# junejunejune/c_orb_slam

Measured on AMD Instinct MI355X. Metric: tracking FPS + ORB matches/sec, KITTI-00 stereo; local-BA iter/sec, higher is better.
Workload: dtype u8

## Files before the change

c_orb_slam_amd/csrc/orb_extract.hip:

```cpp
#include "orb_extract.hpp"

#include <algorithm>
#include <atomic>
#include <chrono>
#include <cmath>
#include <cstring>
#include <thread>

namespace orbgpu {

__constant__ int8_t c_pattern[256 * 4];
__constant__ int8_t c_disc[2 * 1024];
__constant__ int c_ndisc;
__constant__ int c_umax[16];
__constant__ int c_gauss[7];

static const int8_t kPattern[256 * 4] = {
#include "brief_pattern.inc"
};

__device__ __forceinline__ int xcd_tile(int bid, int nb) { return (bid & 7) * (nb >> 3) + (bid >> 3); }
static inline unsigned grid8(int n) { return (unsigned)((n + 7) & ~7); }
constexpr int kFastSplitLevel = 3;

// ... 286 lines not shown
        __syncthreads();
        const int nch = L.pitch >> 4;
        for (int t = tid; t < st.w * nch; t += 256) {
            const int ri = t / nch, ch = t - ri * nch;
            const int py = rl[ri];
            const int y = refl101(py - kEdge, L.h);
            const uint8_t* row = cur + min(max(y - st.x, 0), nrows - 1) * L.rp;
            const int x0 = ch * 16 - kEdge;
            uint4 o;
            if (x0 >= 1 && x0 + 16 <= L.w) {
                const uint32_t* w = reinterpret_cast<const uint32_t*>(row + x0 - 1);
                const uint32_t w0 = w[0], w1 = w[1], w2 = w[2], w3 = w[3], w4 = w[4];
                o.x = __builtin_amdgcn_alignbyte(w1, w0, 1);
                o.y = __builtin_amdgcn_alignbyte(w2, w1, 1);
                o.z = __builtin_amdgcn_alignbyte(w3, w2, 1);
                o.w = __builtin_amdgcn_alignbyte(w4, w3, 1);
            } else {
                uint32_t q[4] = {0, 0, 0, 0};
#pragma unroll
                for (int j = 0; j < 16; j++) q[j >> 2] |= (uint32_t)row[refl101(x0 + j, L.w)] << (8 * (j & 3));
                o = make_uint4(q[0], q[1], q[2], q[3]);
            }
            *reinterpret_cast<uint4*>(base + L.off + (size_t)py * L.pitch + 16 * ch) = o;
        }
        rl += st.w;
        prev = cur;
        prev_lo = st.x;
        prev_rp = L.rp;
        prev_n = nrows;
    }
    (void)src_w;
}

constexpr int BT_W = 128, BT_H = 32, BT_LW = BT_W + 8;
typedef unsigned short ushort2v __attribute__((ext_vector_type(2)));
__device__ __forceinline__ uint32_t dot2u(uint32_t pair, uint32_t taps, uint32_t acc) {
    return __builtin_amdgcn_udot2(__builtin_bit_cast(ushort2v, pair), __builtin_bit_cast(ushort2v, taps), acc, false);
}
__global__ void __launch_bounds__(256) k_blur7(const uint8_t* __restrict__ pyr, uint8_t* __restrict__ blur,
                                               size_t img_bytes, size_t blur_bytes,
                                               const BlurTile* __restrict__ tiles, int ntiles) {
    constexpr int WPR = BT_LW / 4;
    constexpr int SR = BT_H + 6;
    __shared__ uint32_t s_src[SR * WPR];
    __shared__ uint4 s_pair[(SR / 2) * (BT_W / 4)];
    const int tile = xcd_tile(blockIdx.x, gridDim.x);
    if (tile >= ntiles) return;
    const BlurTile tl = tiles[tile];
    const int b = blockIdx.y;
    const uint8_t* P = pyr + (size_t)b * img_bytes + tl.off;
    uint8_t* O = blur + (size_t)b * blur_bytes + tl.boff;
    const int x0 = tl.tx * BT_W, y0 = tl.ty * BT_H;
    {
        constexpr int NU = (SR * WPR + 255) / 256;
        uint32_t v[NU];
#pragma unroll
        for (int u = 0; u < NU; u++) {
            const int i = threadIdx.x + 256 * u;
            const int r = i / WPR, wq = i - r * WPR;
            const int yy = min(y0 + r - 3, tl.h + 2) + kEdge;
            const int c = min(kEdge - 3 + x0 + 4 * wq, tl.pitch - 4);
            v[u] = i < SR * WPR ? *reinterpret_cast<const uint32_t*>(P + (size_t)yy * tl.pitch + c) : 0u;
        }
#pragma unroll
        for (int u = 0; u < NU; u++)
            if (threadIdx.x + 256 * u < SR * WPR) s_src[threadIdx.x + 256 * u] = v[u];
    }
    const uint32_t TLO = (uint32_t)c_gauss[0] | ((uint32_t)c_gauss[1] << 8) | ((uint32_t)c_gauss[2] << 16) |
                         ((uint32_t)c_gauss[3] << 24);
    const uint32_t THI = (uint32_t)c_gauss[4] | ((uint32_t)c_gauss[5] << 8) | ((uint32_t)c_gauss[6] << 16);
    __syncthreads();
    for (int i = threadIdx.x; i < (SR / 2) * (BT_W / 4); i += 256) {
        const int pr = i / (BT_W / 4), q = i - pr * (BT_W / 4);
        uint32_t o[4];
#pragma unroll
        for (int h = 0; h < 2; h++) {
            const uint32_t* w = s_src + (2 * pr + h) * WPR + q;
            const uint32_t w0 = w[0], w1 = w[1], w2 = w[2];
#pragma unroll
            for (int j = 0; j < 4; j++) {
                const uint32_t lo = j ? __builtin_amdgcn_alignbyte(w1, w0, j) : w0;
                const uint32_t hi = j ? __builtin_amdgcn_alignbyte(w2, w1, j) : w1;
                const uint32_t r = __builtin_amdgcn_udot4(lo, TLO, __builtin_amdgcn_udot4(hi, THI, 0u, false), false);
                o[j] = h ? (o[j] | (r << 16)) : r;
            }
        }
        s_pair[i] = make_uint4(o[0], o[1], o[2], o[3]);
    }
    const uint32_t C01 = (uint32_t)c_gauss[0] | ((uint32_t)c_gauss[1] << 16);
    const uint32_t C23 = (uint32_t)c_gauss[2] | ((uint32_t)c_gauss[3] << 16);
    const uint32_t C45 = (uint32_t)c_gauss[4] | ((uint32_t)c_gauss[5] << 16);
    const uint32_t C6_ = (uint32_t)c_gauss[6];
    const uint32_t C_0 = (uint32_t)c_gauss[0] << 16;
    const uint32_t C12 = (uint32_t)c_gauss[1] | ((uint32_t)c_gauss[2] << 16);
    const uint32_t C34 = (uint32_t)c_gauss[3] | ((uint32_t)c_gauss[4] << 16);
    const uint32_t C56 = (uint32_t)c_gauss[5] | ((uint32_t)c_gauss[6] << 16);
    __syncthreads();
    for (int i = threadIdx.x; i < (BT_H / 2) * (BT_W / 4); i += 256) {
        const int p = i / (BT_W / 4), q = i - p * (BT_W / 4);
        const int y = y0 + 2 * p, x = x0 + 4 * q;
        if (y >= tl.h || x >= tl.w) continue;
        const uint4 a = s_pair[(p + 0) * (BT_W / 4) + q], bq = s_pair[(p + 1) * (BT_W / 4) + q];
        const uint4 c = s_pair[(p + 2) * (BT_W / 4) + q], d = s_pair[(p + 3) * (BT_W / 4) + q];
        const uint32_t A[4] = {a.x, a.y, a.z, a.w}, B[4] = {bq.x, bq.y, bq.z, bq.w};
        const uint32_t Cc[4] = {c.x, c.y, c.z, c.w}, D[4] = {d.x, d.y, d.z, d.w};
        uint32_t ev = 0, od = 0;
#pragma unroll
        for (int j = 0; j < 4; j++) {
            const uint32_t se = dot2u(D[j], C6_, dot2u(Cc[j], C45, dot2u(B[j], C23, dot2u(A[j], C01, 0u))));
            const uint32_t so = dot2u(D[j], C56, dot2u(Cc[j], C34, dot2u(B[j], C12, dot2u(A[j], C_0, 0u))));
            ev |= min((se + (1u << 15)) >> 16, 255u) << (8 * j);
            od |= min((so + (1u << 15)) >> 16, 255u) << (8 * j);
        }
        *reinterpret_cast<uint32_t*>(O + (size_t)y * tl.bpitch + x) = ev;
        if (y + 1 < tl.h) *reinterpret_cast<uint32_t*>(O + (size_t)(y + 1) * tl.bpitch + x) = od;
    }
}

constexpr int FC_LD = 76;
constexpr int FC_MAXR = 70;

typedef short short2v __attribute__((ext_vector_type(2)));
__device__ __forceinline__ short2v pk16(int lo, int hi) {
    short2v r;
    r.x = (short)lo;
    r.y = (short)hi;
    return r;
}
__device__ __forceinline__ uint32_t pk_bits(short2v v) { return __builtin_bit_cast(uint32_t, v); }
__device__ __forceinline__ short2v pk_min(short2v a, short2v b) { return __builtin_elementwise_min(a, b); }
__device__ __forceinline__ short2v pk_max(short2v a, short2v b) { return __builtin_elementwise_max(a, b); }

__device__ __forceinline__ short2v fast_score2_lds(const uint8_t* pa, const uint8_t* pb) {
    constexpr int ld = FC_LD;
    constexpr int ring[16] = {3 * ld,      3 * ld + 1,  2 * ld + 2,  ld + 3,  3,  -ld + 3, -2 * ld + 2, -3 * ld + 1,
                              -3 * ld,     -3 * ld - 1, -2 * ld - 2, -ld - 3, -3, ld - 3,  2 * ld - 2,  3 * ld - 1};
    const short2v v = pk16(pa[0], pb[0]);
    short2v d[16], mn2[16], mx2[16];
#pragma unroll
    for (int k = 0; k < 16; k++) d[k] = v - pk16(pa[ring[k]], pb[ring[k]]);
#pragma unroll
    for (int k = 0; k < 16; k++) {
        mn2[k] = pk_min(d[k], d[(k + 1) & 15]);
        mx2[k] = pk_max(d[k], d[(k + 1) & 15]);
    }
    short2v mn4[8], mx4[8];
#pragma unroll
    for (int k = 0; k < 8; k++) {
// ... 395 lines not shown
        scale_[i] = (float)(scale_[i - 1] * scaleFactorD_);
        sigma2_[i] = scale_[i] * scale_[i];
    }
    for (int i = 0; i < nlevels; i++) {
        invScale_[i] = 1.0f / scale_[i];
        invSigma2_[i] = 1.0f / sigma2_[i];
    }
    const float factor = (float)(1.0f / scaleFactorD_);
    float nDesired = nfeatures * (1 - factor) / (1 - (float)std::pow((double)factor, (double)nlevels));
    int sum = 0;
    for (int l = 0; l < nlevels - 1; l++) {
        nPerLevel_[l] = (int)cvRoundf_host(nDesired);
        sum += nPerLevel_[l];
        nDesired *= factor;
    }
    nPerLevel_[nlevels - 1] = std::max(nfeatures - sum, 0);
    umax_.assign(kHalfPatch + 1, 0);
    const int vmax = (int)std::floor(kHalfPatch * std::sqrt(2.f) / 2 + 1);
    const int vmin = (int)std::ceil(kHalfPatch * std::sqrt(2.f) / 2);
    const double hp2 = kHalfPatch * kHalfPatch;
    for (int v = 0; v <= vmax; ++v) umax_[v] = (int)std::lrint(std::sqrt(hp2 - v * v));
    for (int v = kHalfPatch, v0 = 0; v >= vmin; --v) {
        while (umax_[v0] == umax_[v0 + 1]) ++v0;
        umax_[v] = v0;
        ++v0;
    }
}

Extractor::~Extractor() { release(); }

void Extractor::release() {
    release_remap();
    auto F = [](void* p) { if (p) (void)hipFree(p); };
    F(d_in_); F(d_pyr_); F(d_blur_); F(d_slots_); F(d_counts_); F(d_cells_); F(d_tiles_); F(d_work_); F(d_groups_);
    F(d_lcb_); F(d_packed_); F(d_hdr_); F(d_sel_); F(d_levels_); F(d_tabs_);
    F(d_kps_); F(d_desc_); F(d_jobsel_); F(d_jobcnt_); F(d_octlv_); F(d_gscr_); F(d_nout_); F(d_ptiles_);
    F(d_chain_); F(d_cellslot_); F(d_flowcnt_);
    d_flowcnt_ = nullptr;
    d_ptiles_ = nullptr;
    d_chain_ = nullptr;
    d_cellslot_ = nullptr;
    d_jobsel_ = d_jobcnt_ = d_octlv_ = d_gscr_ = d_nout_ = nullptr;
    d_in_ = d_pyr_ = d_blur_ = nullptr;
    d_slots_ = nullptr; d_counts_ = nullptr; d_cells_ = nullptr; d_tiles_ = nullptr; d_work_ = nullptr; d_groups_ = nullptr;
    work_B_ = -1;
    d_lcb_ = nullptr; d_packed_ = nullptr; d_hdr_ = nullptr; d_gtotal_ = nullptr; d_sel_ = nullptr;
    d_levels_ = nullptr; d_tabs_ = nullptr; d_kps_ = nullptr; d_desc_ = nullptr;
    if (h_nout_) (void)hipHostFree(h_nout_);
    h_nout_ = nullptr;
    if (h_in_) (void)hipHostFree(h_in_);
    h_in_ = nullptr;
    h_in_cap_ = 0;
    for (auto& e : ev_) if (e) (void)hipEventDestroy(e);
    for (auto& e : ev_) e = nullptr;
    if (stream_ && ownStream_) (void)hipStreamDestroy(stream_);
    stream_ = nullptr;
    if (evBlur_) (void)hipEventDestroy(evBlur_);
    evBlur_ = nullptr;
    if (evPyrA_) (void)hipEventDestroy(evPyrA_);
    if (evFastA_) (void)hipEventDestroy(evFastA_);
    evPyrA_ = evFastA_ = nullptr;
    if (side_) (void)hipStreamDestroy(side_);
    side_ = nullptr;
}

int Extractor::init_device(int maxW, int maxH, int maxBatch) {
    int ndev = 0;
    if (hipGetDeviceCount(&ndev) != hipSuccess || ndev <= 0) return -4;
    if (const char* pe = getenv("ORBGPU_EXTRACT_STREAM_PRIO"); pe && pe[0] == '1') {
        int lo = 0, hi = 0;
        ORB_HIP_CHECK(hipDeviceGetStreamPriorityRange(&lo, &hi));
        ORB_HIP_CHECK(hipStreamCreateWithPriority(&stream_, hipStreamNonBlocking, hi));
    } else {
        ORB_HIP_CHECK(hipStreamCreateWithFlags(&stream_, hipStreamNonBlocking));
    }
    for (auto& e : ev_) ORB_HIP_CHECK(hipEventCreate(&e));
    const char* eb = getenv("ORBGPU_BLUR_SIDE");
    const char* ef = getenv("ORBGPU_FAST_SPLIT");
    const bool blurSide = eb && atoi(eb) > 0;
    fastSplit_ = ef && atoi(ef) == 1 && !blurSide;
    const char* ew = getenv("ORBGPU_PYR_FLOW");
    flow_ = ew && ew[0] == '1';
    if (blurSide || fastSplit_) ORB_HIP_CHECK(hipStreamCreateWithFlags(&side_, hipStreamNonBlocking));
    if (blurSide) ORB_HIP_CHECK(hipEventCreateWithFlags(&evBlur_, hipEventDisableTiming));
    if (fastSplit_) {
        ORB_HIP_CHECK(hipEventCreateWithFlags(&evPyrA_, hipEventDisableTiming));
        ORB_HIP_CHECK(hipEventCreateWithFlags(&evFastA_, hipEventDisableTiming));
    }
    static bool consts_done = false;
    if (!consts_done) {
        ORB_HIP_CHECK(hipMemcpyToSymbol(HIP_SYMBOL(c_pattern), kPattern, sizeof(kPattern)));
        int taps[7];
        gaussian_taps(taps);
        ORB_HIP_CHECK(hipMemcpyToSymbol(HIP_SYMBOL(c_gauss), taps, sizeof(taps)));
        consts_done = true;
    }
    std::vector<int8_t> disc;
    for (int v = -kHalfPatch; v <= kHalfPatch; v++) {
        const int d = v == 0 ? kHalfPatch : umax_[std::abs(v)];
        for (int u = -d; u <= d; u++) { disc.push_back((int8_t)u); disc.push_back((int8_t)v); }
    }
    const int nd = (int)disc.size() / 2;
    ORB_HIP_CHECK(hipMemcpyToSymbol(HIP_SYMBOL(c_disc), disc.data(), disc.size()));
    ORB_HIP_CHECK(hipMemcpyToSymbol(HIP_SYMBOL(c_ndisc), &nd, sizeof(int)));
    int um[16];
    for (int v = 0; v <= kHalfPatch; v++) um[v] = v == 0 ? kHalfPatch : umax_[v];
    ORB_HIP_CHECK(hipMemcpyToSymbol(HIP_SYMBOL(c_umax), um, sizeof(um)));
    maxW_ = maxW; maxH_ = maxH; maxB_ = maxBatch;
    return 0;
}

int Extractor::build_work(int B) {
    constexpr int kXcds = 8;
    const int ngroups = (int)groups_.size();
    std::vector<int> unit;
    for (int c = 0; c < ngroups; c++)
        if (c == 0 || groups_[c].lvl_off != groups_[c - 1].lvl_off || groups_[c].r0 != groups_[c - 1].r0)
            unit.push_back(c);
    unit.push_back(ngroups);
    const long long splitOff =
        nlevels_ > kFastSplitLevel ? (long long)levels_[kFastSplitLevel].off : std::numeric_limits<long long>::max();
    std::vector<int> work;
    for (int part = 0; part < 2; part++) {
        std::vector<std::vector<int>> lists(kXcds);
        long u = 0;
        for (int b = 0; b < B; b++)
            for (size_t k = 0; k + 1 < unit.size(); k++) {
                if ((groups_[unit[k]].lvl_off < splitOff) != (part == 0)) continue;
                for (int c = unit[k]; c < unit[k + 1]; c++) lists[u % kXcds].push_back((b << 16) | c);
                u++;
            }
        size_t len = 0;
        for (auto& l : lists) len = std::max(len, l.size());
        const size_t base = work.size();
        work.resize(base + len * kXcds, -1);
        for (int x = 0; x < kXcds; x++)
            for (size_t sl = 0; sl < lists[x].size(); sl++) work[base + sl * kXcds + x] = lists[x][sl];
        work_part_[part] = (int)(len * kXcds);
    }
    if (d_work_) (void)hipFree(d_work_);
    d_work_ = nullptr;
    ORB_HIP_CHECK(hipMalloc(&d_work_, std::max<size_t>(work.size(), 1) * 4));
// ... 312 lines not shown
        for (int j = 0; j < ncol;) {
            const CellDesc &a = cells_[cb + j];
            const bool two = j + 1 < ncol && spans(a.c0, a.c1, cells_[cb + j + 1].c0, cells_[cb + j + 1].c1);
            csel.push_back({j, two ? 2 : 1});
            j += two ? 2 : 1;
        }
        for (auto& rp : rsel)
            for (auto& cp : csel) {
                CellGroup g{};
                const CellDesc& tl = cells_[rowb[rp.first] + cp.first];
                const CellDesc& br = cells_[rowb[rp.first + rp.second - 1] + cp.first + cp.second - 1];
                g.r0 = tl.r0; g.c0 = tl.c0;
                g.rows = br.r1 - tl.r0; g.cols = br.c1 - tl.c0;
                g.rsplit = rp.second == 2 ? tl.r1 - tl.r0 - 6 : std::max(g.rows - 6, 0);
                g.csplit = cp.second == 2 ? tl.c1 - tl.c0 - 6 : std::max(g.cols - 6, 0);
                g.pitch = tl.pitch;
                g.lvl_off = tl.lvl_off;
                for (int k = 0; k < 4; k++) {
                    const int di = k >> 1, dj = k & 1;
                    g.cell[k] = -1;
                    if (di >= rp.second || dj >= cp.second) continue;
                    const int c = rowb[rp.first + di] + cp.first + dj;
                    const CellDesc& cd = cells_[c];
                    g.cell[k] = c;
                    g.cap[k] = cd.cap;
                    g.slot_off[k] = cd.slot_off;
                    g.xadd[k] = cd.offx - (cd.c0 - g.c0);
                    g.yadd[k] = cd.offy - (cd.r0 - g.r0);
                }
                groups_.push_back(g);
            }
    }
    if (groups_.size() > 65535) return -1;
    tiles_.clear();
    for (int l = 0; l < nlevels_; l++) {
        const LevelHost& L = levels_[l];
        for (int ty = 0; ty < (L.h + BT_H - 1) / BT_H; ty++)
            for (int tx = 0; tx < (L.w + BT_W - 1) / BT_W; tx++) {
                BlurTile t;
                t.off = L.off; t.pitch = L.pitch; t.w = L.w; t.h = L.h; t.tx = tx; t.ty = ty;
                t.boff = L.boff; t.bpitch = L.bpitch;
                tiles_.push_back(t);
            }
    }
    std::vector<uint8_t> tabs;
    auto push = [&tabs](const void* p, size_t n) -> size_t {
        size_t o = (tabs.size() + 15) & ~(size_t)15;
        tabs.resize(o + n);
        memcpy(tabs.data() + o, p, n);
        return o;
    };
    tab_off_.assign(nlevels_, {0, 0, 0, 0});
    std::vector<std::vector<int>> yrAll(nlevels_);
    xofsAll_.assign(nlevels_, {});
    xalAll_.assign(nlevels_, {});
    ptiles_.clear();
    ptile_begin_.assign(2 * (nlevels_ + 1), 0);
    ptile_n_.assign(2 * nlevels_, 0);
    plds_.assign(2 * nlevels_, 0);
    ptile_th_.assign(2 * nlevels_, 0);
    for (int l = 1; l < nlevels_; l++) {
        const int sw = levels_[l - 1].w, sh = levels_[l - 1].h, dw = levels_[l].w, dh = levels_[l].h;
        const double scale_x = 1. / ((double)dw / sw), scale_y = 1. / ((double)dh / sh);
        std::vector<int> xofs(dw);
        std::vector<short> xal(2 * dw);
        int xmax = dw;
        auto sat_s = [](float v) { long i = std::lrint(v); return (short)std::min(32767L, std::max(-32768L, i)); };
        for (int dx = 0; dx < dw; dx++) {
            float fx = (float)((dx + 0.5) * scale_x - 0.5);
            int sx = (int)std::floor(fx);
            fx -= sx;
            if (sx < 0) { fx = 0; sx = 0; }
            if (sx + 1 >= sw) {
                xmax = std::min(xmax, dx);
                if (sx >= sw - 1) { fx = 0; sx = sw - 1; }
            }
// ... 44 lines not shown
            for (bool ok = false; !ok;) {
                ok = true;
                for (int py0 = 0; py0 < D.ph && ok; py0 += nrow)
                    for (int px0 = 0; px0 < D.pitch && ok; px0 += PT_W) {
                        PyrTile t;
                        ok = make(py0, px0, nrow, t);
                    }
                if (!ok && --nrow < 1) return -1;
            }
            size_t lds = 0;
            for (int py0 = 0; py0 < D.ph; py0 += nrow)
                for (int px0 = 0; px0 < D.pitch; px0 += PT_W) {
                    PyrTile t;
                    make(py0, px0, nrow, t);
                    if ((size_t)(t.sc0 + 4 * t.nsw) > (size_t)levels_[l - 1].pitch) return -1;
                    lds = std::max(lds, (size_t)t.nsr * t.nsw * 4);
                    ptiles_.push_back(t);
                }
            plds_[v * nlevels_ + l] = (int)lds;
            ptile_th_[v * nlevels_ + l] = nrow;
            ptile_n_[v * nlevels_ + l] = (int)ptiles_.size() - ptile_begin_[v * (nlevels_ + 1) + l];
          }
        }
        yrAll[l] = yr;
        xofsAll_[l] = xofs;
        xalAll_[l] = xal;
        tab_off_[l][0] = push(xofs.data(), xofs.size() * 4);
        tab_off_[l][1] = push(xal.data(), xal.size() * 2);
        tab_off_[l][2] = push(yr.data(), yr.size() * 4);
        tab_off_[l][3] = push(yb.data(), yb.size() * 2);
    }
    if (plan_chain(yrAll)) return -1;
    auto F = [](void*& p) { if (p) (void)hipFree(p); p = nullptr; };
    F(d_pyr_); F(d_blur_); F(d_slots_); F(d_counts_); F(d_cells_); F(d_tiles_); F(d_lcb_); F(d_work_); F(d_groups_);
    F(d_cellslot_);
    work_B_ = -1;
    F(d_packed_); F(d_hdr_); F(d_sel_); F(d_levels_); F(d_tabs_); F(d_ptiles_);
    const int B = maxB_;
    if (d_chain_) (void)hipFree(d_chain_);
    d_chain_ = nullptr;
    if (chain_) {
        ORB_HIP_CHECK(hipMalloc(&d_chain_, chainTab_.size()));
        ORB_HIP_CHECK(hipMemcpy(d_chain_, chainTab_.data(), chainTab_.size(), hipMemcpyHostToDevice));
    }
    ORB_HIP_CHECK(hipMalloc(&d_ptiles_, std::max<size_t>(ptiles_.size(), 1) * sizeof(PyrTile)));
    if (!ptiles_.empty())
        ORB_HIP_CHECK(hipMemcpy(d_ptiles_, ptiles_.data(), ptiles_.size() * sizeof(PyrTile), hipMemcpyHostToDevice));
    if (d_flowcnt_) (void)hipFree(d_flowcnt_);
    d_flowcnt_ = nullptr;
    for (int v = 0; v < 2; v++) {
        ptile_th_[v * nlevels_] = kPyrTileH[v];
        int nb = 0, lds = 0;
        for (int l = 0; l < nlevels_; l++) {
            nb += (levels_[l].ph + ptile_th_[v * nlevels_ + l] - 1) / ptile_th_[v * nlevels_ + l];
            lds = std::max(lds, plds_[v * nlevels_ + l]);
        }
        flowBands_[v] = nb;
        flowLds_[v] = lds;
    }
    ORB_HIP_CHECK(hipMalloc(&d_flowcnt_, (size_t)std::max(flowBands_[0], flowBands_[1]) * B * 4));
    ORB_HIP_CHECK(hipMalloc(&d_pyr_, img_bytes_ * B));
    ORB_HIP_CHECK(hipMalloc(&d_blur_, blur_bytes_ * B));
    ORB_HIP_CHECK(hipMemset(d_blur_, 0, blur_bytes_ * B));
    ORB_HIP_CHECK(hipMalloc(&d_slots_, slots_per_image_ * 4 * B));
    ORB_HIP_CHECK(hipMalloc(&d_counts_, cells_.size() * 4 * B));
    ORB_HIP_CHECK(hipMalloc(&d_cells_, cells_.size() * sizeof(CellDesc)));
    ORB_HIP_CHECK(hipMemcpy(d_cells_, cells_.data(), cells_.size() * sizeof(CellDesc), hipMemcpyHostToDevice));
    ORB_HIP_CHECK(hipMalloc(&d_groups_, groups_.size() * sizeof(CellGroup)));
    ORB_HIP_CHECK(hipMemcpy(d_groups_, groups_.data(), groups_.size() * sizeof(CellGroup), hipMemcpyHostToDevice));
    ORB_HIP_CHECK(hipMalloc(&d_tiles_, tiles_.size() * sizeof(BlurTile)));
    ORB_HIP_CHECK(hipMemcpy(d_tiles_, tiles_.data(), tiles_.size() * sizeof(BlurTile), hipMemcpyHostToDevice));
    {
        std::vector<int> cs(cells_.size());
        for (size_t c = 0; c < cells_.size(); c++) cs[c] = cells_[c].slot_off;
        ORB_HIP_CHECK(hipMalloc(&d_cellslot_, std::max<size_t>(cs.size(), 1) * 4));
        ORB_HIP_CHECK(hipMemcpy(d_cellslot_, cs.data(), cs.size() * 4, hipMemcpyHostToDevice));
    }
    ORB_HIP_CHECK(hipMalloc(&d_lcb_, level_cell_begin_.size() * 4));
    ORB_HIP_CHECK(hipMemcpy(d_lcb_, level_cell_begin_.data(), level_cell_begin_.size() * 4, hipMemcpyHostToDevice));
    if (slots_per_image_ * B > ((size_t)1 << 30)) return -1;
    packed_cap_ = (int)(slots_per_image_ * B);
    ORB_HIP_CHECK(hipMalloc(&d_packed_, (size_t)packed_cap_ * 4));
    ORB_HIP_CHECK(hipMalloc(&d_hdr_, (size_t)B * (nlevels_ + 2) * 4 + 64));
    d_gtotal_ = (int*)((char*)d_hdr_ + (size_t)B * (nlevels_ + 2) * 4);
    d_gtotal_alias_ = true;
    sel_cap_ = B * std::max(nfeatures_ * 2 + 64, 256);
    ORB_HIP_CHECK(hipMalloc(&d_sel_, (size_t)sel_cap_ * sizeof(int2)));
    std::vector<LevelDev> ld(nlevels_);
    for (int l = 0; l < nlevels_; l++) {
        ld[l].off = levels_[l].off;
        ld[l].pitch = levels_[l].pitch;
        ld[l].scale = scale_[l];
        ld[l].boff = levels_[l].boff;
        ld[l].bpitch = levels_[l].bpitch;
        ld[l].kp_size = (float)(int)(kPatch * scale_[l]);
    }
    if (nlevels_ > kMaxLevels) return -1;
    for (int l = 0; l < nlevels_; l++) levelArgs_.lv[l] = ld[l];
    ORB_HIP_CHECK(hipMalloc(&d_levels_, ld.size() * sizeof(LevelDev)));
    ORB_HIP_CHECK(hipMemcpy(d_levels_, ld.data(), ld.size() * sizeof(LevelDev), hipMemcpyHostToDevice));
    ORB_HIP_CHECK(hipMalloc(&d_tabs_, std::max<size_t>(tabs.size(), 16)));
    if (!tabs.empty()) ORB_HIP_CHECK(hipMemcpy(d_tabs_, tabs.data(), tabs.size(), hipMemcpyHostToDevice));
    F(d_jobsel_); F(d_jobcnt_); F(d_octlv_); F(d_gscr_); F(d_nout_);
    jcap_ = 0;
// ... 95 lines not shown
                                   img_bytes_, (const CellGroup*)d_groups_, iniTh_, minTh_, (uint32_t*)d_slots_,
                                   slots_per_image_, (int*)d_counts_, ncells, (const int*)d_work_);
                ORB_HIP_CHECK(hipEventRecord(evFastA_, side_));
            }
            const LevelHost& L = levels_[l];
            const LevelHost& P = levels_[l - 1];
            const uint8_t* T = (const uint8_t*)d_tabs_;
            const int v = B >= 8 ? 1 : 0, pb = v * (nlevels_ + 1) + l;
            const int nt = ptile_n_[v * nlevels_ + l];
            auto kern = v ? k_pyr_resize<kPyrTileH[1]> : k_pyr_resize<kPyrTileH[0]>;
            hipLaunchKernelGGL(kern, dim3(grid8(nt), B), dim3(256), plds_[v * nlevels_ + l], s, (uint8_t*)d_pyr_, img_bytes_,
                               P.off, P.pitch, L.off, L.pitch, L.ph, L.w, L.h,
                               (const int*)(T + tab_off_[l][0]), (const short2*)(T + tab_off_[l][1]),
                               (const int2*)(T + tab_off_[l][2]), (const short2*)(T + tab_off_[l][3]),
                               (const PyrTile*)d_ptiles_ + ptile_begin_[pb], nt);
        }
        if (!flow && lend < nlevels_) {
            const uint8_t* T = (const uint8_t*)d_chain_;
            const LevelHost& P = levels_[lend - 1];
            hipLaunchKernelGGL(k_pyr_chain, dim3(chainK_, B), dim3(256), chainLds_, s, (uint8_t*)d_pyr_, img_bytes_,
                               (long long)P.off, P.pitch, P.w, (const ChainLevel*)T, nlevels_ - lend,
                               (const int4*)(T + chainStripOff_), (const uint16_t*)(T + chainRowOff_),
                               (const uint8_t*)d_tabs_, chainSrcLds_, chainSrcRp_);
        }
    }
    ORB_HIP_CHECK(hipGetLastError());
    ORB_HIP_CHECK(hipEventRecord(ev_[1], s));
    static const bool blurEarly = [] {
        const char* e = getenv("ORBGPU_BLUR_EARLY");
        return e && e[0] == '1';
    }();
    if (blurEarly && !evBlur_) {
        planFlags |= kPlanBlurEarly;
        hipLaunchKernelGGL(k_blur7, dim3(grid8((int)tiles_.size()), B), dim3(256), 0, s, (const uint8_t*)d_pyr_,
                           (uint8_t*)d_blur_, img_bytes_, blur_bytes_, (const BlurTile*)d_tiles_, (int)tiles_.size());
    }
    if (evBlur_) {
        ORB_HIP_CHECK(hipStreamWaitEvent(side_, ev_[1], 0));
        hipLaunchKernelGGL(k_blur7, dim3(grid8((int)tiles_.size()), B), dim3(256), 0, side_, (const uint8_t*)d_pyr_,
                           (uint8_t*)d_blur_, img_bytes_, blur_bytes_, (const BlurTile*)d_tiles_, (int)tiles_.size());
        ORB_HIP_CHECK(hipEventRecord(evBlur_, side_));
    }
    if (split) {
        hipLaunchKernelGGL(k_fast_cells, dim3(work_part_[1]), dim3(256), 0, s, (const uint8_t*)d_pyr_, img_bytes_,
                           (const CellGroup*)d_groups_, iniTh_, minTh_, (uint32_t*)d_slots_, slots_per_image_,
                           (int*)d_counts_, ncells, (const int*)d_work_ + work_part_[0]);
        ORB_HIP_CHECK(hipStreamWaitEvent(s, evFastA_, 0));
    } else {
        hipLaunchKernelGGL(k_fast_cells, dim3(work_n_), dim3(256), 0, s, (const uint8_t*)d_pyr_, img_bytes_,
                           (const CellGroup*)d_groups_, iniTh_, minTh_, (uint32_t*)d_slots_, slots_per_image_,
                           (int*)d_counts_, ncells, (const int*)d_work_);
    }
    ORB_HIP_CHECK(hipGetLastError());
    ORB_HIP_CHECK(hipEventRecord(ev_[3], s));
    ORB_HIP_CHECK(hipEventRecord(ev_[4], s));
    int* d_err = (int*)d_nout_ + B;
    OctInput oin{(const uint32_t*)d_slots_, slots_per_image_, (const int*)d_counts_, (const int*)d_cellslot_,
                 (const int*)d_lcb_, ncells, (uint32_t*)d_packed_, d_gtotal_};
    if (int e = octree_launch(oin, B, nlevels_, (const OctLevelDev*)d_octlv_, (uint32_t*)d_jobsel_, (int*)d_jobcnt_,
                              jcap_, (uint16_t*)d_gscr_, (size_t)packed_cap_, cap, (int2*)d_sel_, selcap_,
                              (int*)d_nout_, d_err, s))
        return e;
    ORB_HIP_CHECK(hipEventRecord(ev_[5], s));
    if (evBlur_)
        ORB_HIP_CHECK(hipStreamWaitEvent(s, evBlur_, 0));
    else if (!blurEarly)
        hipLaunchKernelGGL(k_blur7, dim3(grid8((int)tiles_.size()), B), dim3(256), 0, s, (const uint8_t*)d_pyr_,
                           (uint8_t*)d_blur_, img_bytes_, blur_bytes_, (const BlurTile*)d_tiles_, (int)tiles_.size());
    ORB_HIP_CHECK(hipEventRecord(ev_[2], s));
    orb_kp_dev* okps = (orb_kp_dev*)kps;
    uint8_t* odesc = desc;
    if (!out_on_device) {
        const size_t nk = (size_t)B * cap;
        if (nk > out_cap_) {
            if (d_kps_) (void)hipFree(d_kps_);
            if (d_desc_) (void)hipFree(d_desc_);
            ORB_HIP_CHECK(hipMalloc(&d_kps_, nk * sizeof(orb_kp_dev)));
            ORB_HIP_CHECK(hipMalloc(&d_desc_, nk * 32));
            out_cap_ = nk;
        }
        okps = (orb_kp_dev*)d_kps_;
        odesc = (uint8_t*)d_desc_;
    }
    {
        const int gx = (selcap_ + 3) / 4;
        const int nwg = B >= 8 ? gx * 8 * ((B + 7) / 8) : gx * B;
        hipLaunchKernelGGL(k_orient_desc, dim3(nwg), dim3(256), 0, s, (const uint8_t*)d_pyr_,
                           (const uint8_t*)d_blur_, img_bytes_, blur_bytes_, (const int2*)d_sel_, selcap_,
                           (const int*)d_nout_, levelArgs_, okps, odesc, cap, gx, B);
    }
    ORB_HIP_CHECK(hipGetLastError());
    ORB_HIP_CHECK(hipMemcpyAsync(h_nout_, d_nout_, (size_t)(B + 1) * 4, hipMemcpyDeviceToHost, s));
    ORB_HIP_CHECK(hipEventRecord(ev_[6], s));
    ORB_HIP_CHECK(stream_wait(s));
    const int err = h_nout_[B];
    for (int b = 0; b < B; b++) n_out[b] = h_nout_[b];
    if (err & 1) return -3;
    if (err) return -1;
    if (!out_on_device) {
        for (int b = 0; b < B; b++) {
            if (n_out[b] == 0) continue;
// ... 79 lines not shown
```

c_orb_slam_amd/csrc/orb_extract.hpp:

```cpp
#pragma once
#include <atomic>
#include <condition_variable>
#include <cstddef>
#include <cstdint>
#include <mutex>
#include <thread>
#include <vector>
#include <array>

#include "orb_common.hpp"
#include "octree.hpp"
#include "../../include/orbslam_gpu.h"

namespace orbgpu {

struct orb_kp_dev {
    float x, y, size, angle, response;
    int32_t octave, class_id;
};
static_assert(sizeof(orb_kp_dev) == 28, "cv::KeyPoint layout");

struct CellDesc {
    int r0, r1, c0, c1;
    int offx, offy;
    int pitch, cap, slot_off, level;
    long long lvl_off;
};

struct CellGroup {
    int r0, c0, rows, cols;
    int rsplit, csplit;
    int pitch, pad;
    long long lvl_off;
    int cell[4], cap[4], slot_off[4];
    int xadd[4], yadd[4];
};

struct BlurTile {
    long long off, boff;
    int pitch, bpitch, w, h, tx, ty;
};

constexpr int PT_W = 256, kPyrLdsMax = 48 * 1024;
struct PyrTile {
    int py0, px0, nrow, sr0, nsr, sc0, nsw, pad;
};

struct ChainLevel {
    long long off;
    int w, h, pitch, rp, lds, xofs, xal, yr, yb, nph;
};
constexpr int kChainLdsMax = 64 * 1024;

struct FlowLevel {
    long long off;
    int pitch, ph, w, h;
    int task0, ntiles;
    int tile0;
    int band0, th, ncol;
    int xofs, xal, yr, yb;
};
struct FlowArgs {
    FlowLevel L[16];
    int nl, nbands;
};

struct LevelDev {
    long long off, boff;
    int pitch, bpitch;
    float scale, kp_size;
};
constexpr int kMaxLevels = 16;
struct LevelArgs {
// ... 1 lines not shown
};

constexpr int kPlanFlow = 1, kPlanChain = 2, kPlanFastSplit = 4, kPlanBlurSide = 8, kPlanBlurEarly = 16,
              kPlanTile32 = 32;

struct LevelHost {
    int w, h, pw, ph, pitch, bpitch;
    size_t off, boff;
};

class Extractor {
public:
    Extractor(int nfeatures, float scaleFactor, int nlevels, int iniTh, int minTh);
    ~Extractor();
    int init_device(int maxW, int maxH, int maxBatch);
    int extract(const uint8_t* imgs, int B, int W, int H, int step, size_t img_stride, bool imgs_on_device,
                orb_kp* kps, uint8_t* desc, int cap, bool out_on_device, int* n_out,
                const uint8_t* const* list = nullptr);
    int cvt_color(const uint8_t* src, int B, int W, int H, int channels, int rgb, int step, size_t img_stride,
                  bool src_on_device, uint8_t* gray, int gray_step, size_t gray_stride);
    int set_remap(int slot, const float* map1, const float* map2, int W, int H, size_t map_step, bool on_device);
    int remap(const uint8_t* src, int B, int sw, int sh, int step, size_t img_stride, bool src_on_device, int slot0,
              int period, uint8_t* dst, int dst_step, size_t dst_stride);
    bool remap_size(int slot, int* w, int* h) const;
    int get_level(int index, int level, uint8_t* dst, int dst_step, int* w, int* h);
    int get_blurred(int index, int level, uint8_t* dst, int dst_step, int* w, int* h);
    int timings(float* ms6);
    int corner_total(long long* total);
    int last_plan(int* flags, int* chain_from, int* tile_rows) const;
    hipStream_t stream() const { return stream_; }
    int reserve_cus(int one_in_n);
    int share_stream(Extractor* with);
    int build_work(int B);
    const uint8_t* pyramid_base() const { return (const uint8_t*)d_pyr_; }
    size_t pyramid_image_bytes() const { return img_bytes_; }
    const std::vector<LevelHost>& levels() const { return levels_; }
    int last_batch() const { return last_B_; }

    int nlevels() const { return nlevels_; }
    float scale_factor() const { return scaleFactor_; }
    const std::vector<float>& scale() const { return scale_; }
    const std::vector<float>& inv_scale() const { return invScale_; }
    const std::vector<float>& sigma2() const { return sigma2_; }
    const std::vector<float>& inv_sigma2() const { return invSigma2_; }
    const std::vector<int>& n_per_level() const { return nPerLevel_; }

private:
    static void gaussian_taps(int taps[7]);
    int setup_geometry(int W, int H);
    void release();
    int stage_host(const uint8_t* src, size_t need, const uint8_t** dev);
    struct RemapSlot {
        uint16_t* rec = nullptr;
        int w = 0, h = 0, pitch = 0;
    };
    RemapSlot remap_[ORB_REMAP_SLOTS];
    struct Retired {
        void* p;
        bool host;
        hipEvent_t ev;
    };
    std::vector<Retired> retired_;
    int retire(void* p, bool host);
    void sweep_retired(bool wait);
    void release_remap();

    int nfeatures_;
    double scaleFactorD_;
    float scaleFactor_;
    int nlevels_, iniTh_, minTh_;
    std::vector<float> scale_, invScale_, sigma2_, invSigma2_;
    std::vector<int> nPerLevel_, umax_;

    int maxW_ = 0, maxH_ = 0, maxB_ = 0;
    int geomW_ = -1, geomH_ = -1;
    std::vector<LevelHost> levels_;
    LevelArgs levelArgs_{};
    std::vector<CellDesc> cells_;
    std::vector<CellGroup> groups_;
    std::vector<int> level_cell_begin_;
    std::vector<BlurTile> tiles_;
    std::vector<PyrTile> ptiles_;
    std::vector<int> ptile_begin_, ptile_n_, plds_;
    std::vector<int> ptile_th_;
    bool flow_ = false;
    int* d_flowcnt_ = nullptr;
    int flowBands_[2] = {0, 0}, flowLds_[2] = {0, 0};
    FlowArgs flow_args(int v, int B) const;
    int plan_chain(const std::vector<std::vector<int>>& yr);
    bool chain_ = false;
    int chainK_ = 0, chainLds_ = 0, chainFrom_ = 0, chainSrcLds_ = 0, chainSrcRp_ = 0;
    std::vector<std::vector<int>> xofsAll_;
    std::vector<std::vector<short>> xalAll_;
    size_t chainStripOff_ = 0, chainRowOff_ = 0;
    std::vector<uint8_t> chainTab_;
    void* d_chain_ = nullptr;
    void* d_cellslot_ = nullptr;
    std::vector<std::array<size_t, 4>> tab_off_;
    size_t img_bytes_ = 0, blur_bytes_ = 0, slots_per_image_ = 0;
    int packed_cap_ = 0, sel_cap_ = 0;
    int last_B_ = 0;
    int planFlags_ = 0, planChainFrom_ = 0;

    hipStream_t stream_ = nullptr;
    bool ownStream_ = true;
    int lent_ = 0;
    hipEvent_t ev_[7] = {};
    hipStream_t side_ = nullptr;
    hipEvent_t evBlur_ = nullptr;
    bool fastSplit_ = false;
    hipEvent_t evPyrA_ = nullptr, evFastA_ = nullptr;
    void *d_in_ = nullptr, *d_pyr_ = nullptr, *d_blur_ = nullptr, *d_slots_ = nullptr, *d_counts_ = nullptr;
    void *d_ptiles_ = nullptr;
    void *d_cells_ = nullptr, *d_tiles_ = nullptr, *d_lcb_ = nullptr, *d_packed_ = nullptr, *d_hdr_ = nullptr;
    void *d_sel_ = nullptr, *d_levels_ = nullptr, *d_tabs_ = nullptr, *d_kps_ = nullptr, *d_desc_ = nullptr;
    int* d_gtotal_ = nullptr;
    void* d_work_ = nullptr;
    void* d_groups_ = nullptr;
    int work_B_ = -1, work_n_ = 0;
    int work_part_[2] = {0, 0};
    bool d_gtotal_alias_ = false;
    size_t in_cap_ = 0, out_cap_ = 0;
    void* h_in_ = nullptr;
    size_t h_in_cap_ = 0;
    void *d_jobsel_ = nullptr, *d_jobcnt_ = nullptr, *d_octlv_ = nullptr, *d_gscr_ = nullptr, *d_nout_ = nullptr;
    int jcap_ = 0, selcap_ = 0;
    int* h_nout_ = nullptr;

};

int debug_prof_extract(unsigned long long* out32);

}
```

Before: 45350.

## Restructure blur kernel into vertical strips with ring-buffered row pass and prefetch

The 7-tap Gaussian blur now gives each block a full-height 128-wide column strip instead of a 128x32 tile. The block walks down the strip, keeping the horizontal-pass results in an LDS ring buffer so the 6-row halo is not recomputed or reloaded per tile. The next row band is loaded into registers while the current band is computed, and each thread now produces 8 output pixels with wider vector loads and stores. In exchange there are far fewer blocks, which can leave parallelism short on small pyramid levels or small batches, plus extra barriers per step. The grid is also flattened to strips times padded batch.

```diff
diff --git a/c_orb_slam_amd/csrc/orb_extract.hip b/c_orb_slam_amd/csrc/orb_extract.hip
--- a/c_orb_slam_amd/csrc/orb_extract.hip
+++ b/c_orb_slam_amd/csrc/orb_extract.hip
@@ -342,61 +342,75 @@
     (void)src_w;
 }
 
-constexpr int BT_W = 128, BT_H = 32, BT_LW = BT_W + 8;
+constexpr int BT_W = 128, BT_H = 32;
+constexpr int BS_WPR = 36;
+constexpr int BS_SR = BT_H + 6;
+constexpr int BS_RING = BS_SR / 2;
+constexpr int BS_G = BT_W / 8;
 typedef unsigned short ushort2v __attribute__((ext_vector_type(2)));
 __device__ __forceinline__ uint32_t dot2u(uint32_t pair, uint32_t taps, uint32_t acc) {
     return __builtin_amdgcn_udot2(__builtin_bit_cast(ushort2v, pair), __builtin_bit_cast(ushort2v, taps), acc, false);
 }
-__global__ void __launch_bounds__(256) k_blur7(const uint8_t* __restrict__ pyr, uint8_t* __restrict__ blur,
+__device__ __forceinline__ void blur_row_pass(const uint32_t* s_src, uint4* s_pair, int pr, int q8, int slot,
+                                              uint32_t TLO, uint32_t THI) {
+    uint32_t o[8];
+#pragma unroll
+    for (int h = 0; h < 2; h++) {
+        const uint32_t* w = s_src + (2 * pr + h) * BS_WPR + 2 * q8;
+        const uint2 wa = *reinterpret_cast<const uint2*>(w), wb = *reinterpret_cast<const uint2*>(w + 2);
+        const uint32_t W[4] = {wa.x, wa.y, wb.x, wb.y};
+#pragma unroll
+        for (int j = 0; j < 8; j++) {
+            const int d = j >> 2, sh = j & 3;
+            const uint32_t lo = sh ? __builtin_amdgcn_alignbyte(W[d + 1], W[d], sh) : W[d];
+            const uint32_t hi = sh ? __builtin_amdgcn_alignbyte(W[d + 2], W[d + 1], sh) : W[d + 1];
+            const uint32_t r = __builtin_amdgcn_udot4(lo, TLO, __builtin_amdgcn_udot4(hi, THI, 0u, false), false);
+            o[j] = h ? (o[j] | (r << 16)) : r;
+        }
+    }
+    s_pair[slot * (2 * BS_G) + q8] = make_uint4(o[0], o[1], o[2], o[3]);
+    s_pair[slot * (2 * BS_G) + BS_G + q8] = make_uint4(o[4], o[5], o[6], o[7]);
+}
+__global__ void __launch_bounds__(256, 8) k_blur7(const uint8_t* __restrict__ pyr, uint8_t* __restrict__ blur,
                                                size_t img_bytes, size_t blur_bytes,
-                                               const BlurTile* __restrict__ tiles, int ntiles) {
-    constexpr int WPR = BT_LW / 4;
-    constexpr int SR = BT_H + 6;
-    __shared__ uint32_t s_src[SR * WPR];
-    __shared__ uint4 s_pair[(SR / 2) * (BT_W / 4)];
-    const int tile = xcd_tile(blockIdx.x, gridDim.x);
-    if (tile >= ntiles) return;
-    const BlurTile tl = tiles[tile];
-    const int b = blockIdx.y;
-    const uint8_t* P = pyr + (size_t)b * img_bytes + tl.off;
-    uint8_t* O = blur + (size_t)b * blur_bytes + tl.boff;
-    const int x0 = tl.tx * BT_W, y0 = tl.ty * BT_H;
+                                               const BlurStrip* __restrict__ strips, int B, int Bp) {
+    __shared__ __attribute__((aligned(16))) uint32_t s_src[BS_SR * BS_WPR];
+    __shared__ uint4 s_pair[BS_RING * 2 * BS_G];
+    const int k = blockIdx.x / Bp, b = blockIdx.x - k * Bp;
+    if (b >= B) return;
+    const BlurStrip st = strips[k];
+    const uint8_t* P = pyr + (size_t)b * img_bytes + st.off;
+    uint8_t* O = blur + (size_t)b * blur_bytes + st.boff;
+    const int tid = threadIdx.x, x0 = st.tx * BT_W;
+    const int rA = tid >> 3;
+    const int cA = min(kEdge - 3 + x0 + 16 * (tid & 7), st.pitch - 16);
+    const int cT = min(kEdge - 3 + x0 + BT_W, st.pitch - 8);
+    auto row = [&](int y) { return P + (uint32_t)((min(y, st.h + 2) + kEdge) * st.pitch); };
+    uint4 va;
+    uint2 vt = make_uint2(0u, 0u);
+    auto load = [&](int t) {
+        va = *reinterpret_cast<const uint4*>(row(BT_H * t + 3 + rA) + (uint32_t)cA);
+        if (tid < BT_H) vt = *reinterpret_cast<const uint2*>(row(BT_H * t + 3 + tid) + (uint32_t)cT);
+    };
+    auto store = [&]() {
+        *reinterpret_cast<uint4*>(s_src + (6 + rA) * BS_WPR + 4 * (tid & 7)) = va;
+        if (tid < BT_H) *reinterpret_cast<uint2*>(s_src + (6 + tid) * BS_WPR + BT_W / 4) = vt;
+    };
     {
-        constexpr int NU = (SR * WPR + 255) / 256;
-        uint32_t v[NU];
-#pragma unroll
-        for (int u = 0; u < NU; u++) {
-            const int i = threadIdx.x + 256 * u;
-            const int r = i / WPR, wq = i - r * WPR;
-            const int yy = min(y0 + r - 3, tl.h + 2) + kEdge;
-            const int c = min(kEdge - 3 + x0 + 4 * wq, tl.pitch - 4);
-            v[u] = i < SR * WPR ? *reinterpret_cast<const uint32_t*>(P + (size_t)yy * tl.pitch + c) : 0u;
-        }
-#pragma unroll
-        for (int u = 0; u < NU; u++)
-            if (threadIdx.x + 256 * u < SR * WPR) s_src[threadIdx.x + 256 * u] = v[u];
-    }
+        uint4 ea = make_uint4(0u, 0u, 0u, 0u);
+        uint2 et = make_uint2(0u, 0u);
+        if (tid < 6 * 8) ea = *reinterpret_cast<const uint4*>(row(rA - 3) + cA);
+        if (tid < 6) et = *reinterpret_cast<const uint2*>(row(tid - 3) + cT);
+        load(0);
+        if (tid < 6 * 8) *reinterpret_cast<uint4*>(s_src + rA * BS_WPR + 4 * (tid & 7)) = ea;
+        if (tid < 6) *reinterpret_cast<uint2*>(s_src + tid * BS_WPR + BT_W / 4) = et;
+        store();
+    }
+    const int nstep = (st.h + BT_H - 1) / BT_H;
+    if (nstep > 1) load(1);
     const uint32_t TLO = (uint32_t)c_gauss[0] | ((uint32_t)c_gauss[1] << 8) | ((uint32_t)c_gauss[2] << 16) |
                          ((uint32_t)c_gauss[3] << 24);
     const uint32_t THI = (uint32_t)c_gauss[4] | ((uint32_t)c_gauss[5] << 8) | ((uint32_t)c_gauss[6] << 16);
-    __syncthreads();
-    for (int i = threadIdx.x; i < (SR / 2) * (BT_W / 4); i += 256) {
-        const int pr = i / (BT_W / 4), q = i - pr * (BT_W / 4);
-        uint32_t o[4];
-#pragma unroll
-        for (int h = 0; h < 2; h++) {
-            const uint32_t* w = s_src + (2 * pr + h) * WPR + q;
-            const uint32_t w0 = w[0], w1 = w[1], w2 = w[2];
-#pragma unroll
-            for (int j = 0; j < 4; j++) {
-                const uint32_t lo = j ? __builtin_amdgcn_alignbyte(w1, w0, j) : w0;
-                const uint32_t hi = j ? __builtin_amdgcn_alignbyte(w2, w1, j) : w1;
-                const uint32_t r = __builtin_amdgcn_udot4(lo, TLO, __builtin_amdgcn_udot4(hi, THI, 0u, false), false);
-                o[j] = h ? (o[j] | (r << 16)) : r;
-            }
-        }
-        s_pair[i] = make_uint4(o[0], o[1], o[2], o[3]);
-    }
     const uint32_t C01 = (uint32_t)c_gauss[0] | ((uint32_t)c_gauss[1] << 16);
     const uint32_t C23 = (uint32_t)c_gauss[2] | ((uint32_t)c_gauss[3] << 16);
     const uint32_t C45 = (uint32_t)c_gauss[4] | ((uint32_t)c_gauss[5] << 16);
@@ -405,25 +419,57 @@
     const uint32_t C12 = (uint32_t)c_gauss[1] | ((uint32_t)c_gauss[2] << 16);
     const uint32_t C34 = (uint32_t)c_gauss[3] | ((uint32_t)c_gauss[4] << 16);
     const uint32_t C56 = (uint32_t)c_gauss[5] | ((uint32_t)c_gauss[6] << 16);
+    const int p = tid / BS_G, q8 = tid - p * BS_G;
+    const int x = x0 + 8 * q8;
     __syncthreads();
-    for (int i = threadIdx.x; i < (BT_H / 2) * (BT_W / 4); i += 256) {
-        const int p = i / (BT_W / 4), q = i - p * (BT_W / 4);
-        const int y = y0 + 2 * p, x = x0 + 4 * q;
-        if (y >= tl.h || x >= tl.w) continue;
-        const uint4 a = s_pair[(p + 0) * (BT_W / 4) + q], bq = s_pair[(p + 1) * (BT_W / 4) + q];
-        const uint4 c = s_pair[(p + 2) * (BT_W / 4) + q], d = s_pair[(p + 3) * (BT_W / 4) + q];
-        const uint32_t A[4] = {a.x, a.y, a.z, a.w}, B[4] = {bq.x, bq.y, bq.z, bq.w};
-        const uint32_t Cc[4] = {c.x, c.y, c.z, c.w}, D[4] = {d.x, d.y, d.z, d.w};
-        uint32_t ev = 0, od = 0;
-#pragma unroll
-        for (int j = 0; j < 4; j++) {
-            const uint32_t se = dot2u(D[j], C6_, dot2u(Cc[j], C45, dot2u(B[j], C23, dot2u(A[j], C01, 0u))));
-            const uint32_t so = dot2u(D[j], C56, dot2u(Cc[j], C34, dot2u(B[j], C12, dot2u(A[j], C_0, 0u))));
-            ev |= min((se + (1u << 15)) >> 16, 255u) << (8 * j);
-            od |= min((so + (1u << 15)) >> 16, 255u) << (8 * j);
-        }
-        *reinterpret_cast<uint32_t*>(O + (size_t)y * tl.bpitch + x) = ev;
-        if (y + 1 < tl.h) *reinterpret_cast<uint32_t*>(O + (size_t)(y + 1) * tl.bpitch + x) = od;
+    for (int i = tid; i < BS_RING * BS_G; i += 256) blur_row_pass(s_src, s_pair, i / BS_G, i % BS_G, i / BS_G, TLO, THI);
+    __syncthreads();
+    int base = 0;
+    for (int s = 0; s < nstep; s++) {
+        const int y = BT_H * s + 2 * p;
+        const bool out = y < st.h && x < st.w;
+        uint32_t ev[2] = {0u, 0u}, od[2] = {0u, 0u};
+        if (out) {
+            int sl[4];
+#pragma unroll
+            for (int c = 0; c < 4; c++) {
+                sl[c] = base + p + c;
+                sl[c] = (sl[c] >= BS_RING ? sl[c] - BS_RING : sl[c]) * (2 * BS_G) + q8;
+            }
+#pragma unroll
+            for (int hf = 0; hf < 2; hf++) {
+                const uint4 a = s_pair[sl[0] + hf * BS_G], bq = s_pair[sl[1] + hf * BS_G];
+                const uint4 c = s_pair[sl[2] + hf * BS_G], d = s_pair[sl[3] + hf * BS_G];
+                const uint32_t A[4] = {a.x, a.y, a.z, a.w}, Bq[4] = {bq.x, bq.y, bq.z, bq.w};
+                const uint32_t Cc[4] = {c.x, c.y, c.z, c.w}, D[4] = {d.x, d.y, d.z, d.w};
+                uint32_t e = 0, o = 0;
+#pragma unroll
+                for (int j = 0; j < 4; j++) {
+                    const uint32_t se = dot2u(D[j], C6_, dot2u(Cc[j], C45, dot2u(Bq[j], C23, dot2u(A[j], C01, 1u << 15))));
+                    const uint32_t so = dot2u(D[j], C56, dot2u(Cc[j], C34, dot2u(Bq[j], C12, dot2u(A[j], C_0, 1u << 15))));
+                    e |= min(se >> 16, 255u) << (8 * j);
+                    o |= min(so >> 16, 255u) << (8 * j);
+                }
+                ev[hf] = e;
+                od[hf] = o;
+            }
+        }
+        if (s + 1 < nstep) store();
+        if (s + 2 < nstep) load(s + 2);
+        if (out) {
+            const uint32_t oo = (uint32_t)(y * st.bpitch + x);
+            *reinterpret_cast<uint2*>(O + oo) = make_uint2(ev[0], ev[1]);
+            if (y + 1 < st.h) *reinterpret_cast<uint2*>(O + oo + (uint32_t)st.bpitch) = make_uint2(od[0], od[1]);
+        }
+        if (s + 1 == nstep) break;
+        base = base + 16 >= BS_RING ? base + 16 - BS_RING : base + 16;
+        __syncthreads();
+        {
+            const int pr = 3 + p;
+            const int sl = base + pr >= BS_RING ? base + pr - BS_RING : base + pr;
+            blur_row_pass(s_src, s_pair, pr, q8, sl, TLO, THI);
+        }
+        __syncthreads();
     }
 }
 
@@ -885,7 +931,7 @@
 void Extractor::release() {
     release_remap();
     auto F = [](void* p) { if (p) (void)hipFree(p); };
-    F(d_in_); F(d_pyr_); F(d_blur_); F(d_slots_); F(d_counts_); F(d_cells_); F(d_tiles_); F(d_work_); F(d_groups_);
+    F(d_in_); F(d_pyr_); F(d_blur_); F(d_slots_); F(d_counts_); F(d_cells_); F(d_strips_); F(d_work_); F(d_groups_);
     F(d_lcb_); F(d_packed_); F(d_hdr_); F(d_sel_); F(d_levels_); F(d_tabs_);
     F(d_kps_); F(d_desc_); F(d_jobsel_); F(d_jobcnt_); F(d_octlv_); F(d_gscr_); F(d_nout_); F(d_ptiles_);
     F(d_chain_); F(d_cellslot_); F(d_flowcnt_);
@@ -895,7 +941,7 @@
     d_cellslot_ = nullptr;
     d_jobsel_ = d_jobcnt_ = d_octlv_ = d_gscr_ = d_nout_ = nullptr;
     d_in_ = d_pyr_ = d_blur_ = nullptr;
-    d_slots_ = nullptr; d_counts_ = nullptr; d_cells_ = nullptr; d_tiles_ = nullptr; d_work_ = nullptr; d_groups_ = nullptr;
+    d_slots_ = nullptr; d_counts_ = nullptr; d_cells_ = nullptr; d_strips_ = nullptr; d_work_ = nullptr; d_groups_ = nullptr;
     work_B_ = -1;
     d_lcb_ = nullptr; d_packed_ = nullptr; d_hdr_ = nullptr; d_gtotal_ = nullptr; d_sel_ = nullptr;
     d_levels_ = nullptr; d_tabs_ = nullptr; d_kps_ = nullptr; d_desc_ = nullptr;
@@ -961,6 +1007,12 @@
     ORB_HIP_CHECK(hipMemcpyToSymbol(HIP_SYMBOL(c_umax), um, sizeof(um)));
     maxW_ = maxW; maxH_ = maxH; maxB_ = maxBatch;
     return 0;
+}
+
+void Extractor::launch_blur(int B, hipStream_t s) {
+    const int Bp = B >= 8 ? (B + 7) & ~7 : B;
+    hipLaunchKernelGGL(k_blur7, dim3((unsigned)strips_.size() * Bp), dim3(256), 0, s, (const uint8_t*)d_pyr_,
+                       (uint8_t*)d_blur_, img_bytes_, blur_bytes_, (const BlurStrip*)d_strips_, B, Bp);
 }
 
 int Extractor::build_work(int B) {
@@ -1339,16 +1391,15 @@
             }
     }
     if (groups_.size() > 65535) return -1;
-    tiles_.clear();
+    strips_.clear();
     for (int l = 0; l < nlevels_; l++) {
         const LevelHost& L = levels_[l];
-        for (int ty = 0; ty < (L.h + BT_H - 1) / BT_H; ty++)
-            for (int tx = 0; tx < (L.w + BT_W - 1) / BT_W; tx++) {
-                BlurTile t;
-                t.off = L.off; t.pitch = L.pitch; t.w = L.w; t.h = L.h; t.tx = tx; t.ty = ty;
-                t.boff = L.boff; t.bpitch = L.bpitch;
-                tiles_.push_back(t);
-            }
+        for (int tx = 0; tx < (L.w + BT_W - 1) / BT_W; tx++) {
+            BlurStrip t{};
+            t.off = L.off; t.pitch = L.pitch; t.w = L.w; t.h = L.h; t.tx = tx;
+            t.boff = L.boff; t.bpitch = L.bpitch;
+            strips_.push_back(t);
+        }
     }
     std::vector<uint8_t> tabs;
     auto push = [&tabs](const void* p, size_t n) -> size_t {
@@ -1459,7 +1510,7 @@
     }
     if (plan_chain(yrAll)) return -1;
     auto F = [](void*& p) { if (p) (void)hipFree(p); p = nullptr; };
-    F(d_pyr_); F(d_blur_); F(d_slots_); F(d_counts_); F(d_cells_); F(d_tiles_); F(d_lcb_); F(d_work_); F(d_groups_);
+    F(d_pyr_); F(d_blur_); F(d_slots_); F(d_counts_); F(d_cells_); F(d_strips_); F(d_lcb_); F(d_work_); F(d_groups_);
     F(d_cellslot_);
     work_B_ = -1;
     F(d_packed_); F(d_hdr_); F(d_sel_); F(d_levels_); F(d_tabs_); F(d_ptiles_);
@@ -1495,8 +1546,8 @@
     ORB_HIP_CHECK(hipMemcpy(d_cells_, cells_.data(), cells_.size() * sizeof(CellDesc), hipMemcpyHostToDevice));
     ORB_HIP_CHECK(hipMalloc(&d_groups_, groups_.size() * sizeof(CellGroup)));
     ORB_HIP_CHECK(hipMemcpy(d_groups_, groups_.data(), groups_.size() * sizeof(CellGroup), hipMemcpyHostToDevice));
-    ORB_HIP_CHECK(hipMalloc(&d_tiles_, tiles_.size() * sizeof(BlurTile)));
-    ORB_HIP_CHECK(hipMemcpy(d_tiles_, tiles_.data(), tiles_.size() * sizeof(BlurTile), hipMemcpyHostToDevice));
+    ORB_HIP_CHECK(hipMalloc(&d_strips_, strips_.size() * sizeof(BlurStrip)));
+    ORB_HIP_CHECK(hipMemcpy(d_strips_, strips_.data(), strips_.size() * sizeof(BlurStrip), hipMemcpyHostToDevice));
     {
         std::vector<int> cs(cells_.size());
         for (size_t c = 0; c < cells_.size(); c++) cs[c] = cells_[c].slot_off;
@@ -1658,13 +1709,11 @@
     }();
     if (blurEarly && !evBlur_) {
         planFlags |= kPlanBlurEarly;
-        hipLaunchKernelGGL(k_blur7, dim3(grid8((int)tiles_.size()), B), dim3(256), 0, s, (const uint8_t*)d_pyr_,
-                           (uint8_t*)d_blur_, img_bytes_, blur_bytes_, (const BlurTile*)d_tiles_, (int)tiles_.size());
+        launch_blur(B, s);
     }
     if (evBlur_) {
         ORB_HIP_CHECK(hipStreamWaitEvent(side_, ev_[1], 0));
-        hipLaunchKernelGGL(k_blur7, dim3(grid8((int)tiles_.size()), B), dim3(256), 0, side_, (const uint8_t*)d_pyr_,
-                           (uint8_t*)d_blur_, img_bytes_, blur_bytes_, (const BlurTile*)d_tiles_, (int)tiles_.size());
+        launch_blur(B, side_);
         ORB_HIP_CHECK(hipEventRecord(evBlur_, side_));
     }
     if (split) {
@@ -1691,8 +1740,7 @@
     if (evBlur_)
         ORB_HIP_CHECK(hipStreamWaitEvent(s, evBlur_, 0));
     else if (!blurEarly)
-        hipLaunchKernelGGL(k_blur7, dim3(grid8((int)tiles_.size()), B), dim3(256), 0, s, (const uint8_t*)d_pyr_,
-                           (uint8_t*)d_blur_, img_bytes_, blur_bytes_, (const BlurTile*)d_tiles_, (int)tiles_.size());
+        launch_blur(B, s);
     ORB_HIP_CHECK(hipEventRecord(ev_[2], s));
     orb_kp_dev* okps = (orb_kp_dev*)kps;
     uint8_t* odesc = desc;
diff --git a/c_orb_slam_amd/csrc/orb_extract.hpp b/c_orb_slam_amd/csrc/orb_extract.hpp
--- a/c_orb_slam_amd/csrc/orb_extract.hpp
+++ b/c_orb_slam_amd/csrc/orb_extract.hpp
@@ -36,9 +36,9 @@
     int xadd[4], yadd[4];
 };
 
-struct BlurTile {
+struct BlurStrip {
     long long off, boff;
-    int pitch, bpitch, w, h, tx, ty;
+    int pitch, bpitch, w, h, tx, pad;
 };
 
 constexpr int PT_W = 256, kPyrLdsMax = 48 * 1024;
@@ -106,6 +106,7 @@
     int reserve_cus(int one_in_n);
     int share_stream(Extractor* with);
     int build_work(int B);
+    void launch_blur(int B, hipStream_t s);
     const uint8_t* pyramid_base() const { return (const uint8_t*)d_pyr_; }
     size_t pyramid_image_bytes() const { return img_bytes_; }
     const std::vector<LevelHost>& levels() const { return levels_; }
@@ -153,7 +154,7 @@
     std::vector<CellDesc> cells_;
     std::vector<CellGroup> groups_;
     std::vector<int> level_cell_begin_;
-    std::vector<BlurTile> tiles_;
+    std::vector<BlurStrip> strips_;
     std::vector<PyrTile> ptiles_;
     std::vector<int> ptile_begin_, ptile_n_, plds_;
     std::vector<int> ptile_th_;
@@ -186,7 +187,7 @@
     hipEvent_t evPyrA_ = nullptr, evFastA_ = nullptr;
     void *d_in_ = nullptr, *d_pyr_ = nullptr, *d_blur_ = nullptr, *d_slots_ = nullptr, *d_counts_ = nullptr;
     void *d_ptiles_ = nullptr;
-    void *d_cells_ = nullptr, *d_tiles_ = nullptr, *d_lcb_ = nullptr, *d_packed_ = nullptr, *d_hdr_ = nullptr;
+    void *d_cells_ = nullptr, *d_strips_ = nullptr, *d_lcb_ = nullptr, *d_packed_ = nullptr, *d_hdr_ = nullptr;
     void *d_sel_ = nullptr, *d_levels_ = nullptr, *d_tabs_ = nullptr, *d_kps_ = nullptr, *d_desc_ = nullptr;
     int* d_gtotal_ = nullptr;
     void* d_work_ = nullptr;
```

Measured after the change: 46540, median of 5. 1.03x the previous value.
